# Vasilispapg/CVML-GoalNet

Measured on AMD Instinct MI355X. Metric: training clips/sec at batch 64, 16-frame 224² clips; logit MAE vs CPU ref, higher is better.
Workload: dtype f32; 1 GPU; AVM train step (forward + broadcast-MSE + backward + fused Adam), 64 clips x 16 frames = 1024 frames of 3x224x224 + 30x30 MFCC per GPU; dropout live (device masks), BatchNorm train mode; frames_per_gpu=1024, h=224, w=224, parallelism=dp1, ddp_semantics=local BN + local MSE per rank, gradient mean (standard DDP), params=1286754369

## Files before the change

cvml_goalnet_amd/csrc/gemm_f32.hip:

```cpp
#include <stdlib.h>

#include "gemm_common.h"
#include "skinny.h"

using namespace goalnet;

namespace {

constexpr int BM = 128, BN = 128, BK = 32;
constexpr int LDR = 128;
constexpr int OP_FLOATS = BM * BK;

__device__ __forceinline__ int kc_off(int row, int chunk) { return row * BK + ((chunk ^ ((row >> 1) & 7)) << 2); }

__device__ __forceinline__ float4 f4zero() { return make_float4(0.f, 0.f, 0.f, 0.f); }
__device__ __forceinline__ float4 f4fma(float4 v, float4 s, float4 t) {
    return make_float4(fmaf(v.x, s.x, t.x), fmaf(v.y, s.y, t.y), fmaf(v.z, s.z, t.z), fmaf(v.w, s.w, t.w));
}

typedef unsigned int u32x4 __attribute__((ext_vector_type(4)));
constexpr unsigned OOB = 0xFFFFFF00u;

__device__ __forceinline__ float4 f4sel(bool v, float4 a) { return v ? a : f4zero(); }

__device__ __forceinline__ __amdgpu_buffer_rsrc_t make_rsrc(const void* base, uint32_t bytes) {
    return __builtin_amdgcn_make_buffer_rsrc(const_cast<void*>(base), 0, (int)bytes, 0x00020000);
}
__device__ __forceinline__ float4 bload(__amdgpu_buffer_rsrc_t r, unsigned voff, unsigned soff) {
    const u32x4 v = __builtin_amdgcn_raw_buffer_load_b128(r, (int)voff, (int)soff, 0);
    return make_float4(__uint_as_float(v.x), __uint_as_float(v.y), __uint_as_float(v.z), __uint_as_float(v.w));
}
__device__ __forceinline__ uint32_t clamp_u32(int64_t v) {
    return v <= 0 ? 0u : (v > 0xFFFFFF00ll ? 0xFFFFFF00u : (uint32_t)v);
}

template <bool AFFINE>
struct KCLoader {
    struct P {
        const float* x; int64_t ld; int rows;
        const float* scale; const float* shift; int bnC;
        int convC;
    };
    static constexpr bool KC = true;
    static constexpr bool ONE_STAGE = false;
    static constexpr int ONE_STAGE_BLOCKS = 3;
    __amdgpu_buffer_rsrc_t rx, rsc, rsh;
    unsigned voff[4], vaff;
    int bnC, convC;
    float4 sc, sh;
    __device__ KCLoader(const P& p, int row0, int tid) {
        const int nrows = p.rows - row0 < BM ? p.rows - row0 : BM;
        rx = make_rsrc(p.x + (int64_t)row0 * p.ld, clamp_u32((int64_t)nrows * p.ld * 4));
#pragma unroll
        for (int i = 0; i < 4; ++i) {
            const int rl = (tid >> 3) + 32 * i;
            voff[i] = rl < nrows ? (unsigned)(((int64_t)rl * p.ld + (tid & 7) * 4) * 4) : OOB;
        }
        bnC = p.bnC; convC = p.convC;
        if (AFFINE) {
            rsc = make_rsrc(p.scale, (uint32_t)p.bnC * 4);
            rsh = make_rsrc(p.shift, (uint32_t)p.bnC * 4);
            vaff = (unsigned)((tid & 7) * 16);
        }
    }
    __device__ __forceinline__ void issue(int kt, float4 (&r)[4]) {
        unsigned k4 = (unsigned)kt * (BK * 4);
        if (convC > 0) {
            const int chunk = kt / 9, tap = kt - 9 * chunk;
            k4 = (unsigned)(tap * convC + chunk * BK) * 4;
        }
        if (AFFINE) {
            const unsigned ch4 = (unsigned)((kt * BK) % bnC) * 4;
            sc = bload(rsc, vaff, ch4);
            sh = bload(rsh, vaff, ch4);
        }
#pragma unroll
        for (int i = 0; i < 4; ++i) r[i] = bload(rx, voff[i], k4);
    }
    __device__ __forceinline__ void finish(float4 (&r)[4]) const {
        if (AFFINE) {
#pragma unroll
            for (int i = 0; i < 4; ++i) r[i] = f4fma(r[i], sc, sh);
        }
    }
};

template <bool AFFINE>
struct MCLoader {
    struct P {
        const float* x; int64_t ld; int cols; int kred;
        const float* scale; const float* shift; int bnC;
    };
    static constexpr bool KC = false;
    static constexpr bool ONE_STAGE = true;
#ifndef GN_MC_BLOCKS
#define GN_MC_BLOCKS 4
#endif
    static constexpr int ONE_STAGE_BLOCKS = GN_MC_BLOCKS;
    const float* x;
    int64_t ld;
    int kred, k0;
    unsigned voff[4];
    bool partial;
    float4 sc, sh;
    __device__ MCLoader(const P& p, int col0, int tid) {
        const int col = col0 + (tid & 31) * 4;
        const bool colok = col < p.cols;
        x = p.x; ld = p.ld; kred = p.kred; k0 = tid >> 5;
#pragma unroll
        for (int i = 0; i < 4; ++i) voff[i] = colok ? (unsigned)(((int64_t)(k0 + 8 * i) * p.ld + col) * 4) : OOB;
        partial = false;
        if (AFFINE) {
            const int ch = (colok ? col : 0) % p.bnC;
            sc = *reinterpret_cast<const float4*>(p.scale + ch);
            sh = *reinterpret_cast<const float4*>(p.shift + ch);
            if (!colok) sh = f4zero();
        }
    }
    __device__ __forceinline__ void issue(int kt, float4 (&r)[4]) {
        const int kbase = kt * BK;
        const int nk = kred - kbase < BK ? kred - kbase : BK;
        partial = nk < BK;
        const __amdgpu_buffer_rsrc_t rx = make_rsrc(x + (int64_t)kbase * ld, clamp_u32((int64_t)nk * ld * 4));
#pragma unroll
        for (int i = 0; i < 4; ++i) r[i] = bload(rx, voff[i], 0);
    }
    __device__ __forceinline__ void finish(float4 (&r)[4]) const {
        if (AFFINE) {
            if (partial) {
#pragma unroll
                for (int i = 0; i < 4; ++i) r[i] = f4sel(k0 + 8 * i < (kred & (BK - 1)), f4fma(r[i], sc, sh));
            } else {
#pragma unroll
                for (int i = 0; i < 4; ++i) r[i] = f4fma(r[i], sc, sh);
            }
        }
    }
};

template <bool AFFINE>
struct ConvALoader {
    struct P {
        const float* x; int H, W, C; int64_t M;
        const float* scale; const float* shift;
    };
    static constexpr bool KC = true;
    static constexpr bool ONE_STAGE = true;
    static constexpr int ONE_STAGE_BLOCKS = AFFINE ? 3 : 4;
    __amdgpu_buffer_rsrc_t rx, rsc, rsh;
    unsigned mask[4];
    unsigned voff, vaff, vmask;
    int W, C;
    float4 sc, sh;
    __device__ ConvALoader(const P& p, int row0, int tid) {
        W = p.W; C = p.C;
        const int c4 = (tid & 7) * 4, rr = tid >> 3;
        rx = make_rsrc(p.x + ((int64_t)row0 - (p.W + 1)) * p.C, (uint32_t)((BM + 2 * (p.W + 1)) * p.C * 4));
        voff = (unsigned)((rr * p.C + c4) * 4);
        if (AFFINE) {
            rsc = make_rsrc(p.scale, (uint32_t)p.C * 4);
            rsh = make_rsrc(p.shift, (uint32_t)p.C * 4);
            vaff = (unsigned)(c4 * 4);
        }
#pragma unroll
        for (int i = 0; i < 4; ++i) {
            const int64_t m = (int64_t)row0 + rr + 32 * i;
            unsigned mk = 0;
            if (m < p.M) {
                const int w = (int)((unsigned)m % (unsigned)p.W);
                const int h = (int)(((unsigned)m / (unsigned)p.W) % (unsigned)p.H);
#pragma unroll
                for (int kh = 0; kh < 3; ++kh)
#pragma unroll
                    for (int kw = 0; kw < 3; ++kw) {
                        const bool v = (unsigned)(h + kh - 1) < (unsigned)p.H && (unsigned)(w + kw - 1) < (unsigned)p.W;
                        mk |= (v ? 1u : 0u) << (kh * 3 + kw);
                    }
            }
            mask[i] = mk;
        }
    }
    __device__ __forceinline__ void issue(int kt, float4 (&r)[4]) {
        const int chunk = kt / 9;
        const int tap = kt - 9 * chunk;
        const int ci = chunk * BK;
        const int kh = tap / 3, kw = tap - 3 * kh;
        const unsigned s0 = (unsigned)(((kh * W + kw) * C + ci) * 4);
        const unsigned rowstep = (unsigned)(32 * C * 4);
        if (AFFINE) {
            sc = bload(rsc, vaff, (unsigned)ci * 4);
            sh = bload(rsh, vaff, (unsigned)ci * 4);
        }
        vmask = 0;
#pragma unroll
        for (int i = 0; i < 4; ++i) {
            const bool v = (mask[i] >> tap) & 1u;
            vmask |= (v ? 1u : 0u) << i;
            r[i] = bload(rx, v ? voff : OOB, s0 + (unsigned)i * rowstep);
        }
    }
    __device__ __forceinline__ void finish(float4 (&r)[4]) const {
        if (AFFINE) {
#pragma unroll
            for (int i = 0; i < 4; ++i) r[i] = f4sel((vmask >> i) & 1u, f4fma(r[i], sc, sh));
        }
    }
};

template <bool AFFINE, bool DSEL = false>
struct ConvWgradBLoader {
    struct P {
        const float* x; int H, W, C; int M;
        const float* scale; const float* shift;
        const uint32_t* codes4;
    };
    static constexpr bool KC = false;
    const float* x;
    __amdgpu_buffer_rsrc_t rcodes;
    int W, C, M, k0, tapshift, nextkt;
    unsigned voff[4], bad4, nextcode, badnow;
    float4 sc, sh;
    __device__ ConvWgradBLoader(const P& p, int col0, int tid) {
        const int col = col0 + (tid & 31) * 4;
        const bool colok = col < 9 * p.C;
        const int cc = colok ? col : 0;
        const int tap = cc / p.C, ci = cc - tap * p.C;
        const int kh = tap / 3, kw = tap - 3 * kh;
        x = p.x; W = p.W; C = p.C; M = p.M; k0 = tid >> 5;
        rcodes = make_rsrc(p.codes4, (uint32_t)((p.M + 31) / 32 * 32));
        bad4 = ((kh == 0 ? 1u : 0u) | (kh == 2 ? 2u : 0u) | (kw == 0 ? 4u : 0u) | (kw == 2 ? 8u : 0u)) * 0x01010101u;
        tapshift = kh * p.W + kw;
        nextkt = -1; nextcode = 0;
#pragma unroll
        for (int i = 0; i < 4; ++i) voff[i] = colok ? (unsigned)(((k0 + 8 * i + tapshift) * p.C + ci) * 4) : OOB;
        if (AFFINE) {
            sc = *reinterpret_cast<const float4*>(p.scale + ci);
            sh = *reinterpret_cast<const float4*>(p.shift + ci);
        }
    }
    __device__ __forceinline__ unsigned load_code(int kt) const {
        return (unsigned)__builtin_amdgcn_raw_buffer_load_b32(rcodes, k0 * 4, kt * 32, 0);
    }
    __device__ __forceinline__ void issue(int kt, float4 (&r)[4]) {
        const int mbase = kt * BK;
        const unsigned badc = (nextkt == kt ? nextcode : load_code(kt)) & bad4;
        badnow = badc;
        const unsigned bad = DSEL ? 0u : badc;
        const int64_t lead = (int64_t)mbase - (W + 1);
        const int64_t last = (int64_t)mbase + BK + (W + 1) < M ? (int64_t)mbase + BK + (W + 1) : M;
        const __amdgpu_buffer_rsrc_t rx = make_rsrc(x + lead * C, clamp_u32((last - lead) * C * 4));
        if (lead < 0) {
#pragma unroll
            for (int i = 0; i < 4; ++i)
                r[i] = bload(rx, (mbase + k0 + 8 * i + tapshift < W + 1 || ((bad >> (8 * i)) & 0xFFu)) ? OOB : voff[i], 0);
        } else {
#pragma unroll
            for (int i = 0; i < 4; ++i) r[i] = bload(rx, ((bad >> (8 * i)) & 0xFFu) ? OOB : voff[i], 0);
        }
        nextcode = load_code(kt + 1);
        nextkt = kt + 1;
    }
    __device__ __forceinline__ void finish(float4 (&r)[4]) const {
        if (DSEL) {
#pragma unroll
            for (int i = 0; i < 4; ++i) r[i] = f4sel(((badnow >> (8 * i)) & 0xFFu) == 0, AFFINE ? f4fma(r[i], sc, sh) : r[i]);
        } else if (AFFINE) {
#pragma unroll
            for (int i = 0; i < 4; ++i) r[i] = f4fma(r[i], sc, sh);
        }
    }
};

__global__ __launch_bounds__(256) void border_codes_kernel(uint32_t* __restrict__ codes4, int M, int Mpad, int H, int W) {
    for (int j = blockIdx.x * blockDim.x + threadIdx.x; j < Mpad / 4; j += gridDim.x * blockDim.x) {
        const int kt = j >> 3, k0 = j & 7;
        uint32_t word = 0;
#pragma unroll
        for (int i = 0; i < 4; ++i) {
            const int m = kt * 32 + k0 + 8 * i;
            const int w = m % W, h = (m / W) % H;
            const uint32_t c = m < M ? (uint32_t)((h == 0 ? 1 : 0) | (h == H - 1 ? 2 : 0) | (w == 0 ? 4 : 0) | (w == W - 1 ? 8 : 0)) : 0xFu;
            word |= c << (8 * i);
        }
        codes4[j] = word;
    }
}

__global__ __launch_bounds__(256) void wgrad_border_sums_kernel(const float* __restrict__ dy, double* __restrict__ parts,
                                                               int H, int W, int Cout) {
    const int n = blockIdx.x;
    const float* f = dy + (int64_t)n * H * W * Cout;
    double* out = parts + (int64_t)n * 8 * Cout;
    for (int c = threadIdx.x; c < Cout; c += blockDim.x) {
        double r0 = 0, r1 = 0, c0 = 0, c1 = 0;
        for (int w = 0; w < W; ++w) { r0 += (double)f[(int64_t)w * Cout + c]; r1 += (double)f[((int64_t)(H - 1) * W + w) * Cout + c]; }
        for (int h = 0; h < H; ++h) { c0 += (double)f[(int64_t)h * W * Cout + c]; c1 += (double)f[((int64_t)h * W + W - 1) * Cout + c]; }
        out[0 * Cout + c] = r0; out[1 * Cout + c] = r1; out[2 * Cout + c] = c0; out[3 * Cout + c] = c1;
        out[4 * Cout + c] = (double)f[c];
        out[5 * Cout + c] = (double)f[(int64_t)(W - 1) * Cout + c];
        out[6 * Cout + c] = (double)f[(int64_t)(H - 1) * W * Cout + c];
        out[7 * Cout + c] = (double)f[((int64_t)(H - 1) * W + W - 1) * Cout + c];
    }
}

__device__ __forceinline__ float border_u_of(const double* v, int tap) {
    const int kh = tap / 3, kw = tap - 3 * kh;
    double r = (kh == 0 ? v[0] : 0.0) + (kh == 2 ? v[1] : 0.0) + (kw == 0 ? v[2] : 0.0) + (kw == 2 ? v[3] : 0.0);
    if (kh == 0 && kw == 0) r -= v[4];
    if (kh == 0 && kw == 2) r -= v[5];
    if (kh == 2 && kw == 0) r -= v[6];
    if (kh == 2 && kw == 2) r -= v[7];
    return (float)r;
}

__global__ __launch_bounds__(256) void wgrad_border_u_kernel(const double* __restrict__ parts, int N, int Cout, float* __restrict__ u) {
    __shared__ double s[32][8];
    const int cl = threadIdx.x & 31, j = threadIdx.x >> 5;
    const int c = blockIdx.x * 32 + cl;
    double a0 = 0, a1 = 0, a2 = 0, a3 = 0;
    if (c < Cout) {
        const double* q = parts + (int64_t)j * Cout + c;
        int n = 0;
        for (; n + 3 < N; n += 4) {
            a0 += q[(int64_t)n * 8 * Cout]; a1 += q[(int64_t)(n + 1) * 8 * Cout];
            a2 += q[(int64_t)(n + 2) * 8 * Cout]; a3 += q[(int64_t)(n + 3) * 8 * Cout];
        }
        for (; n < N; ++n) a0 += q[(int64_t)n * 8 * Cout];
    }
    s[cl][j] = (a0 + a1) + (a2 + a3);
    __syncthreads();
    for (int t = threadIdx.x; t < 32 * 9; t += 256) {
        const int cc = t / 9, tap = t - 9 * cc;
        if (blockIdx.x * 32 + cc < Cout) u[(int64_t)(blockIdx.x * 32 + cc) * 9 + tap] = border_u_of(s[cc], tap);
    }
}

template <bool KC>
__device__ __forceinline__ void store_tile(float* l, const float4 (&r)[4], int tid) {
    if (KC) {
        const int c4 = (tid & 7) * 4, row = tid >> 3;
#pragma unroll
        for (int i = 0; i < 4; ++i) *reinterpret_cast<float4*>(&l[kc_off(row + 32 * i, c4 >> 2)]) = r[i];
    } else {
        const int r4 = (tid & 31) * 4, k = tid >> 5;
#pragma unroll
        for (int i = 0; i < 4; ++i) *reinterpret_cast<float4*>(&l[(k + 8 * i) * LDR + r4]) = r[i];
    }
}

template <bool KC>
__device__ __forceinline__ void read_group(const float* l, int strip, int s, int r, int h, float (&f)[2][4]) {
    if (KC) {
#pragma unroll
        for (int q = 0; q < 2; ++q) {
            const float4 t = *reinterpret_cast<const float4*>(&l[kc_off(strip + q * 32 + r, 2 * s + h)]);
            f[q][0] = t.x; f[q][1] = t.y; f[q][2] = t.z; f[q][3] = t.w;
        }
    } else {
#pragma unroll
        for (int j = 0; j < 4; ++j) {
            const float2 t = *reinterpret_cast<const float2*>(&l[(8 * s + 4 * h + j) * LDR + strip + 2 * r]);
            f[0][j] = t.x; f[1][j] = t.y;
        }
    }
}

template <bool AKC, bool BKC>
__device__ __forceinline__ void compute_tile(const float* la, const float* lb, f32x16 (&acc)[2][2],
                                             int wm, int wn, int r, int h) {
#pragma unroll
    for (int s = 0; s < 4; ++s) {
        float a[2][4], b[2][4];
        read_group<AKC>(la, wm * 64, s, r, h, a);
        read_group<BKC>(lb, wn * 64, s, r, h, b);
#pragma unroll
        for (int j = 0; j < 4; ++j) {
#pragma unroll
            for (int fm = 0; fm < 2; ++fm)
#pragma unroll
                for (int fn = 0; fn < 2; ++fn)
                    acc[fm][fn] = __builtin_amdgcn_mfma_f32_32x32x2f32(a[fm][j], b[fn][j], acc[fm][fn], 0, 0, 0);
        }
    }
}

__device__ __forceinline__ void compute_tile_n64(const float* la, const float* lb, f32x16 (&acc)[2], int wave, int r, int h) {
#pragma unroll
    for (int s = 0; s < 4; ++s) {
        const float4 ta = *reinterpret_cast<const float4*>(&la[kc_off(wave * 32 + r, 2 * s + h)]);
        const float4 tb0 = *reinterpret_cast<const float4*>(&lb[kc_off(r, 2 * s + h)]);
        const float4 tb1 = *reinterpret_cast<const float4*>(&lb[kc_off(32 + r, 2 * s + h)]);
        const float a[4] = {ta.x, ta.y, ta.z, ta.w}, b0[4] = {tb0.x, tb0.y, tb0.z, tb0.w}, b1[4] = {tb1.x, tb1.y, tb1.z, tb1.w};
#pragma unroll
        for (int j = 0; j < 4; ++j) {
            acc[0] = __builtin_amdgcn_mfma_f32_32x32x2f32(a[j], b0[j], acc[0], 0, 0, 0);
            acc[1] = __builtin_amdgcn_mfma_f32_32x32x2f32(a[j], b1[j], acc[1], 0, 0, 0);
        }
    }
}

__device__ __forceinline__ void store_acc_n64(const EpiP& ep, const f32x16 (&acc)[2], int tm, int tn, int split, int wave, int r, int h) {
    float* outp = ep.slab_stride > 0 ? (ep.slabs ? ep.slabs : ep.out) + (int64_t)split * ep.slab_stride : ep.out;
    const int mode = ep.slab_stride > 0 ? EPI_RAW : ep.mode;
    const int64_t ld = (ep.slab_stride > 0 && ep.slabs) ? (int64_t)ep.cols : ep.ld;
#pragma unroll
    for (int fn = 0; fn < 2; ++fn) {
        const int col = tn * 64 + fn * 32 + r;
        const bool colok = col < ep.cols;
        const int64_t row0 = (int64_t)tm * BM + wave * 32 + 4 * h;
        const float bv = (mode == EPI_BIAS_RELU && ep.bias) ? ep.bias[colok ? col : 0] : 0.f;
        const float lo = (mode == EPI_BIAS_RELU && ep.relu) ? 0.f : -INFINITY;
#pragma unroll
        for (int e = 0; e < 16; ++e) {
            const int64_t row = row0 + (e & 3) + 8 * (e >> 2);
            if (!(colok && row < ep.rows)) continue;
            const float v = acc[fn][e];
            if (mode == EPI_RAW) outp[row * ld + col] = v;
            else if (mode == EPI_BIAS_RELU) outp[row * ld + col] = fmaxf(v + bv, lo);
            else outp[row * ld + col] = epi_apply(ep, v, row, col);
        }
    }
}

template <class AL, class BL, bool N64 = false, int STAGES = 2>
__global__ __launch_bounds__(256, STAGES == 1 ? (N64 ? 4 : AL::ONE_STAGE_BLOCKS) : 2) void gemm_f32_kernel(typename AL::P ap, typename BL::P bp, EpiP ep,
                                                          int tiles_m, int tiles_n, int m_fast,
                                                          int ktiles, int ktiles_per_split, int xcd_splits) {
    __shared__ __attribute__((aligned(16))) float lds[STAGES][2][OP_FLOATS];
    const int tid = threadIdx.x;
    int tm, tn, split;
    if (xcd_splits > 0) {
        const int tiles = tiles_m * tiles_n;
        const int xcd = blockIdx.x & 7, j = blockIdx.x >> 3;
        int t;
        if (tiles > 64 && tiles <= 128) {
            const int gs = (xcd_splits + 7) / 8, rest = tiles - 64, nA = gs * 64;
            int q;
            if (j < nA) { q = j >> 6; t = j & 63; }
            else { const int i = j - nA; q = i / rest; t = 64 + (i - q * rest); }
            split = q * 8 + xcd;
        } else {
            split = (j / tiles) * 8 + xcd;
            t = j - (j / tiles) * tiles;
        }
        if (split >= xcd_splits) return;
        if (m_fast) { tm = t % tiles_m; tn = t / tiles_m; } else { tn = t % tiles_n; tm = t / tiles_n; }
    } else {
        tile_of_block(tiles_m, tiles_n, m_fast, tm, tn);
        split = blockIdx.y;
    }
    const int kt0 = split * ktiles_per_split;
    const int kt1 = min(ktiles, kt0 + ktiles_per_split);

    static_assert(!N64 || (AL::KC && BL::KC), "the 128 x 64 tile reads K-contiguous LDS images");
    AL al(ap, tm * BM, tid);
    BL bl(bp, tn * (N64 ? 64 : BN), tid);

    const int lane = tid & 63, wave = tid >> 6;
    const int wm = wave >> 1, wn = wave & 1;
    const int r = lane & 31, h = lane >> 5;

    f32x16 acc[2][2];
#pragma unroll
    for (int i = 0; i < 2; ++i)
#pragma unroll
        for (int j = 0; j < 2; ++j)
#pragma unroll
            for (int e = 0; e < 16; ++e) acc[i][j][e] = 0.f;

    float4 ra[4], rb[4];
    if (kt0 < kt1) {
        al.issue(kt0, ra);
        bl.issue(kt0, rb);
        al.finish(ra);
        bl.finish(rb);
        store_tile<AL::KC>(lds[0][0], ra, tid);
        store_tile<BL::KC>(lds[0][1], rb, tid);
    }
    __syncthreads();
    for (int kt = kt0; kt < kt1; ++kt) {
        const int cur = STAGES == 1 ? 0 : (kt - kt0) & 1;
        const bool more = kt + 1 < kt1;
        if (more) {
            al.issue(kt + 1, ra);
            bl.issue(kt + 1, rb);
        }
        if constexpr (N64) compute_tile_n64(lds[cur][0], lds[cur][1], acc[0], wave, r, h);
        else compute_tile<AL::KC, BL::KC>(lds[cur][0], lds[cur][1], acc, wm, wn, r, h);
        if constexpr (STAGES == 1) __syncthreads();
        if (more) {
            al.finish(ra);
            bl.finish(rb);
            store_tile<AL::KC>(lds[STAGES == 1 ? 0 : cur ^ 1][0], ra, tid);
            store_tile<BL::KC>(lds[STAGES == 1 ? 0 : cur ^ 1][1], rb, tid);
        }
        __syncthreads();
    }
    if constexpr (N64) store_acc_n64(ep, acc[0], tm, tn, split, wave, r, h);
    else store_acc<!AL::KC, !BL::KC>(ep, acc, tm, tn, split, wm, wn, r, h);
    if (ep.tile_ctr) {
        const int nsp = (ktiles + ktiles_per_split - 1) / ktiles_per_split;
        fused_splitk_reduce<N64 ? 64 : BN>(ep, tm, tn, tm * tiles_n + tn, nsp, tid);
    }
}

__global__ __launch_bounds__(256) void splitk_reduce_kernel(const float* slabs, int nsplit, int64_t slab_stride, EpiP ep) {
    const int c4n = ep.cols >> 2;
    const int64_t total = (int64_t)ep.rows * c4n;
    for (int64_t i = (int64_t)blockIdx.x * blockDim.x + threadIdx.x; i < total; i += (int64_t)gridDim.x * blockDim.x) {
        const int64_t row = i / c4n;
        const int col = (int)(i - row * c4n) * 4;
        const float* s = slabs + row * ep.cols + col;
        float4 a = *reinterpret_cast<const float4*>(s);
        for (int k = 1; k < nsplit; ++k) {
            const float4 b = *reinterpret_cast<const float4*>(s + (int64_t)k * slab_stride);
            a.x += b.x; a.y += b.y; a.z += b.z; a.w += b.w;
        }
        if (ep.oscale) { const int k = *ep.oscale; a.x = ldexpf(a.x, k); a.y = ldexpf(a.y, k); a.z = ldexpf(a.z, k); a.w = ldexpf(a.w, k); }
        if (ep.corr_u) {
            const int tap = col / ep.corr_C, ci = col - tap * ep.corr_C;
            const float u = ep.corr_u[row * 9 + tap];
            const float4 shv = *reinterpret_cast<const float4*>(ep.corr_sh + ci);
            a.x = fmaf(-shv.x, u, a.x); a.y = fmaf(-shv.y, u, a.y); a.z = fmaf(-shv.z, u, a.z); a.w = fmaf(-shv.w, u, a.w);
        }
        float* o = ep.out + row * ep.ld + col;
        o[0] = epi_apply(ep, a.x, row, col);
        o[1] = epi_apply(ep, a.y, row, col + 1);
        o[2] = epi_apply(ep, a.z, row, col + 2);
        o[3] = epi_apply(ep, a.w, row, col + 3);
    }
}

__global__ __launch_bounds__(256) void splitk_reduce_wide_kernel(const float* slabs, int nsplit, int64_t slab_stride, EpiP ep) {
    const int c4n = ep.cols >> 2;
    const int64_t total = (int64_t)ep.rows * c4n;
    const int g = threadIdx.x & 15;
    const int64_t step = (int64_t)gridDim.x * 16;
    const int64_t rounds = (total + step - 1) / step;
    int64_t i = (int64_t)blockIdx.x * 16 + (threadIdx.x >> 4);
    for (int64_t r = 0; r < rounds; ++r, i += step) {
        const bool ok = i < total;
        const int64_t ic = ok ? i : 0;
        const int64_t row = ic / c4n;
        const int col = (int)(ic - row * c4n) * 4;
        const float* s = slabs + row * ep.cols + col;
        float4 a = make_float4(0.f, 0.f, 0.f, 0.f);
        for (int k = g; k < nsplit; k += 16) {
            const float4 b = *reinterpret_cast<const float4*>(s + (int64_t)k * slab_stride);
            a.x += b.x; a.y += b.y; a.z += b.z; a.w += b.w;
        }
        a.x = row16_sum(a.x); a.y = row16_sum(a.y); a.z = row16_sum(a.z); a.w = row16_sum(a.w);
        if (ep.oscale) { const int k = *ep.oscale; a.x = ldexpf(a.x, k); a.y = ldexpf(a.y, k); a.z = ldexpf(a.z, k); a.w = ldexpf(a.w, k); }
        if (ep.corr_u) {
            const int tap = col / ep.corr_C, ci = col - tap * ep.corr_C;
            const float u = ep.corr_u[row * 9 + tap];
            const float4 shv = *reinterpret_cast<const float4*>(ep.corr_sh + ci);
            a.x = fmaf(-shv.x, u, a.x); a.y = fmaf(-shv.y, u, a.y); a.z = fmaf(-shv.z, u, a.z); a.w = fmaf(-shv.w, u, a.w);
        }
        if (ok && g == 0) {
            float* o = ep.out + row * ep.ld + col;
            o[0] = epi_apply(ep, a.x, row, col);
            o[1] = epi_apply(ep, a.y, row, col + 1);
            o[2] = epi_apply(ep, a.z, row, col + 2);
            o[3] = epi_apply(ep, a.w, row, col + 3);
        }
    }
}

template <class AL, class BL, bool N64 = false>
int launch_gemm(const char* name, const typename AL::P& ap, const typename BL::P& bp, const EpiP& ep,
                int64_t M, int64_t N, int ktiles, int nsplit, int m_fast, hipStream_t st) {
    const int64_t tiles_m = (M + BM - 1) / BM, tiles_n = (N + (N64 ? 64 : BN) - 1) / (N64 ? 64 : BN);
    GN_REQUIRE(tiles_m * tiles_n < (1ll << 31), GOALNET_E_SHAPE, "%s: too many tiles", name);
    GN_REQUIRE(nsplit >= 1 && nsplit <= 65535, GOALNET_E_SHAPE, "%s: bad split count %d", name, nsplit);
    const int kps = (ktiles + nsplit - 1) / nsplit;
    GN_REQUIRE(!ep.tile_ctr || (ktiles + kps - 1) / kps == nsplit, GOALNET_E_SHAPE, "%s: fused split-K needs every split non-empty", name);
    const bool xcd_local = nsplit >= 8 && tiles_m * tiles_n <= 256 && tiles_m * tiles_n * ((nsplit + 7) / 8 * 8) < (1ll << 31);
    dim3 grid((unsigned)(tiles_m * tiles_n), (unsigned)nsplit, 1);
    if (xcd_local) grid = dim3((unsigned)(tiles_m * tiles_n * ((nsplit + 7) / 8 * 8)), 1, 1);
    static const int force_stages = getenv("GOALNET_F32_STAGES") ? atoi(getenv("GOALNET_F32_STAGES")) : 0;
    const bool one_stage = force_stages == 1 || (force_stages != 2 && AL::ONE_STAGE);
    if (one_stage) {
        hipLaunchKernelGGL((gemm_f32_kernel<AL, BL, N64, 1>), grid, dim3(256), 0, st, ap, bp, ep, (int)tiles_m, (int)tiles_n,
                           m_fast, ktiles, kps, xcd_local ? nsplit : 0);
        GN_LAUNCH_CHECK(name);
        return 0;
    }
    hipLaunchKernelGGL((gemm_f32_kernel<AL, BL, N64>), grid, dim3(256), 0, st, ap, bp, ep, (int)tiles_m, (int)tiles_n,
                       m_fast, ktiles, kps, xcd_local ? nsplit : 0);
    GN_LAUNCH_CHECK(name);
    return 0;
}

}

namespace goalnet {
int launch_splitk_reduce(const char* name, const float* slabs, int nsplit, int64_t slab_stride, const EpiP& ep, hipStream_t st) {
    const int64_t total = (int64_t)ep.rows * (ep.cols >> 2);
    int64_t blocks = (total + 255) / 256;
    if (blocks > 4096) blocks = 4096;
    if (blocks < 1) blocks = 1;
    if (total < 65536 && nsplit >= 32) {
        int64_t wb = (total + 15) / 16;
        if (wb > 4096) wb = 4096;
        hipLaunchKernelGGL(splitk_reduce_wide_kernel, dim3((unsigned)wb), dim3(256), 0, st, slabs, nsplit, slab_stride, ep);
        GN_LAUNCH_CHECK(name);
        return 0;
    }
    hipLaunchKernelGGL(splitk_reduce_kernel, dim3((unsigned)blocks), dim3(256), 0, st, slabs, nsplit, slab_stride, ep);
    GN_LAUNCH_CHECK(name);
    return 0;
}

int pick_splits(int64_t tiles, int ktiles) {
    if (ktiles < 8 || (ktiles < 64 && tiles >= 128)) return 1;
    int64_t s = ((ktiles < 64 ? 256 : 1024) + tiles - 1) / tiles;
    const int64_t smax = ktiles < 64 ? ktiles / 4 : (ktiles / 8 > 1 ? ktiles / 8 : 1);
    if (s > smax) s = smax;
    if (s < 1) s = 1;
    const int kps = (int)((ktiles + s - 1) / s);
    return (ktiles + kps - 1) / kps;
}

}

extern "C" {

static int conv_splits_f32(int64_t M, int Cin, int Cout) {
    return conv_fwd_splits(((M + BM - 1) / BM) * ((Cout + BN - 1) / BN), 9 * Cin / BK);
}

size_t goalnet_conv3x3_fwd_ws_bytes(int N, int H, int W, int Cin, int Cout) {
    if (N <= 0 || H <= 0 || W <= 0 || Cin <= 0 || Cout <= 0) return 0;
    const int64_t M = (int64_t)N * H * W;
    const int s = conv_splits_f32(M, Cin, Cout);
    return s > 1 ? (size_t)s * (size_t)M * (size_t)Cout * sizeof(float) : 0;
}

int goalnet_conv3x3_fwd(const float* x, const float* scale, const float* shift, const float* w,
                        const float* bias, int relu, float* y, int N, int H, int W, int Cin, int Cout,
                        void* ws, size_t ws_bytes, int* tile_ctr, int n_ctr, void* stream) {
    GN_REQUIRE(x && w && y, GOALNET_E_NULL, "conv3x3_fwd: null pointer");
    GN_REQUIRE((scale == nullptr) == (shift == nullptr), GOALNET_E_NULL, "conv3x3_fwd: scale/shift must both be set or both NULL");
    GN_REQUIRE(N > 0 && H > 0 && W > 0 && Cin > 0 && Cout > 0, GOALNET_E_SHAPE, "conv3x3_fwd: non-positive dim");
    GN_REQUIRE(Cin % BK == 0, GOALNET_E_SHAPE, "conv3x3_fwd: Cin=%d must be a multiple of %d", Cin, BK);
    GN_REQUIRE(Cout % 4 == 0, GOALNET_E_SHAPE, "conv3x3_fwd: Cout=%d must be a multiple of 4", Cout);
    GN_REQUIRE(aligned16(x) && aligned16(w) && aligned16(y) && aligned16(scale) && aligned16(shift),
               GOALNET_E_ALIGN, "conv3x3_fwd: pointers must be 16-byte aligned");
    const int64_t M = (int64_t)N * H * W;
    GN_REQUIRE(M < (1ll << 31) - 256, GOALNET_E_SHAPE, "conv3x3_fwd: N*H*W too large");
    hipStream_t st = (hipStream_t)stream;
    KCLoader<false>::P bp{w, (int64_t)9 * Cin, Cout, nullptr, nullptr, 1, Cin};
    const EpiP efinal{EPI_BIAS_RELU, y, Cout, (int)M, Cout, bias, relu, nullptr, 0, nullptr, 0, 0};
    EpiP ep = efinal;
    const int ktiles = 9 * Cin / BK;
    int nsplit = ws ? conv_splits_f32(M, Cin, Cout) : 1;
    if (nsplit > 1) {
        GN_REQUIRE(aligned16(ws) && ws_bytes >= goalnet_conv3x3_fwd_ws_bytes(N, H, W, Cin, Cout), GOALNET_E_WORKSPACE,
                   "conv3x3_fwd: workspace too small or misaligned");
        ep = EpiP{EPI_RAW, (float*)ws, Cout, (int)M, Cout, nullptr, 0, nullptr, 0, nullptr, 0, M * Cout};
    }
    const bool narrow = Cout <= 64 && !getenv("GOALNET_F32_N64_OFF");
    const bool fused = nsplit > 1 && tile_ctr && (int64_t)n_ctr >= ((M + BM - 1) / BM) * ((Cout + (narrow ? 64 : BN) - 1) / (narrow ? 64 : BN));
    if (fused) {
        ep = efinal;
        ep.slabs = (float*)ws; ep.slab_stride = M * Cout; ep.tile_ctr = tile_ctr;
    }
    int rc;
    if (scale) {
        ConvALoader<true>::P ap{x, H, W, Cin, M, scale, shift};
        rc = narrow ? launch_gemm<ConvALoader<true>, KCLoader<false>, true>("conv3x3_fwd", ap, bp, ep, M, Cout, ktiles, nsplit, 0, st)
                    : launch_gemm<ConvALoader<true>, KCLoader<false>>("conv3x3_fwd", ap, bp, ep, M, Cout, ktiles, nsplit, 0, st);
    } else {
        ConvALoader<false>::P ap{x, H, W, Cin, M, nullptr, nullptr};
        rc = narrow ? launch_gemm<ConvALoader<false>, KCLoader<false>, true>("conv3x3_fwd", ap, bp, ep, M, Cout, ktiles, nsplit, 0, st)
                    : launch_gemm<ConvALoader<false>, KCLoader<false>>("conv3x3_fwd", ap, bp, ep, M, Cout, ktiles, nsplit, 0, st);
    }
    if (rc || nsplit == 1 || fused) return rc;
    return launch_splitk_reduce("conv3x3_fwd.reduce", (const float*)ws, nsplit, M * Cout, efinal, st);
}

}
namespace {
template <class AL, class BL, bool N64, int STAGES> const char* gemm_f32_kernel_name_() { return __PRETTY_FUNCTION__; }
template <class AL, class BL, bool N64> const char* gemm_f32_kernel_name() {
    const int force = getenv("GOALNET_F32_STAGES") ? atoi(getenv("GOALNET_F32_STAGES")) : 0;
    const bool one = force == 1 || (force != 2 && AL::ONE_STAGE);
    return one ? gemm_f32_kernel_name_<AL, BL, N64, 1>() : gemm_f32_kernel_name_<AL, BL, N64, 2>();
}
}
extern "C" {

const char* goalnet_conv3x3_fwd_kernel_name(int N, int H, int W, int Cin, int Cout, int affine) {
    (void)N; (void)H; (void)W; (void)Cin;
    const bool narrow = Cout <= 64 && !getenv("GOALNET_F32_N64_OFF");
    if (affine) return narrow ? gemm_f32_kernel_name<ConvALoader<true>, KCLoader<false>, true>() : gemm_f32_kernel_name<ConvALoader<true>, KCLoader<false>, false>();
    return narrow ? gemm_f32_kernel_name<ConvALoader<false>, KCLoader<false>, true>() : gemm_f32_kernel_name<ConvALoader<false>, KCLoader<false>, false>();
}

static int wgrad_splits(int64_t M, int Cin, int Cout) {
    const int64_t tiles = (int64_t)((Cout + BM - 1) / BM) * ((9 * Cin + BN - 1) / BN);
    const int ktiles = (int)((M + BK - 1) / BK);
    static const int wtarget = getenv("GOALNET_WGRAD_SPLIT_TARGET") ? atoi(getenv("GOALNET_WGRAD_SPLIT_TARGET")) : 2048;
    int64_t s = (wtarget + tiles - 1) / tiles;
    const int64_t smax = ktiles / 4 > 1 ? ktiles / 4 : 1;
    if (s > smax) s = smax;
    if (s > 512) s = 512;
    if (s >= 8) {
        int64_t best = (s + 7) / 8 * 8 <= smax ? (s + 7) / 8 * 8 : s / 8 * 8;
        double best_eff = 0.0;
        for (int64_t c = best; c <= 2 * s + 8 && c <= smax && c <= 1024; c += 8) {
            const int64_t blocks = tiles * c, rounds = (blocks + 511) / 512;
            const double eff = (double)blocks / (double)(rounds * 512);
            if (eff > best_eff + 1e-9) { best_eff = eff; best = c; }
        }
        s = best;
    }
    const int kps = (int)((ktiles + s - 1) / s);
    return (ktiles + kps - 1) / kps;
}

static size_t wgrad_codes_bytes(int64_t M) { return (size_t)((M + 31) / 32 * 32 + 255) / 256 * 256; }
static size_t wgrad_border_bytes(int N, int Cout) {
    return ((size_t)N * 8 * Cout * sizeof(double) + 255) / 256 * 256 + ((size_t)Cout * 9 * sizeof(float) + 255) / 256 * 256;
}

size_t goalnet_conv3x3_wgrad_ws_bytes(int N, int H, int W, int Cin, int Cout) {
    const int64_t M = (int64_t)N * H * W;
    return wgrad_codes_bytes(M) + wgrad_border_bytes(N, Cout) + (size_t)wgrad_splits(M, Cin, Cout) * (size_t)Cout * 9 * Cin * sizeof(float);
}

int goalnet_conv3x3_wgrad_codes(uint32_t* codes, int N, int H, int W, void* stream) {
    GN_REQUIRE(codes && N > 0 && H > 0 && W > 0, GOALNET_E_NULL, "conv3x3_wgrad_codes: bad arguments");
    const int64_t M = (int64_t)N * H * W;
    GN_REQUIRE(M < (1ll << 31) - 256, GOALNET_E_SHAPE, "conv3x3_wgrad_codes: N*H*W too large");
    const int Mpad = (int)((M + 31) / 32 * 32);
    int blocks = (Mpad / 4 + 255) / 256;
    if (blocks > 4096) blocks = 4096;
    hipLaunchKernelGGL(border_codes_kernel, dim3(blocks), dim3(256), 0, (hipStream_t)stream, codes, (int)M, Mpad, H, W);
    GN_LAUNCH_CHECK("conv3x3_wgrad_codes");
    return 0;
}

size_t goalnet_conv3x3_wgrad_codes_bytes(int N, int H, int W) { return wgrad_codes_bytes((int64_t)N * H * W); }

int goalnet_conv3x3_wgrad(const float* x, const float* scale, const float* shift, const float* dy, float* dw,
                          void* ws, size_t ws_bytes, const uint32_t* codes_in, int* tile_ctr, int n_ctr,
                          int N, int H, int W, int Cin, int Cout, void* stream) {
    GN_REQUIRE(x && dy && dw && ws, GOALNET_E_NULL, "conv3x3_wgrad: null pointer");
    GN_REQUIRE((scale == nullptr) == (shift == nullptr), GOALNET_E_NULL, "conv3x3_wgrad: scale/shift must both be set or both NULL");
    GN_REQUIRE(N > 0 && H > 0 && W > 0, GOALNET_E_SHAPE, "conv3x3_wgrad: non-positive dim");
    GN_REQUIRE(Cin % 4 == 0 && Cout % 4 == 0 && Cin > 0 && Cout > 0, GOALNET_E_SHAPE, "conv3x3_wgrad: channels must be multiples of 4");
    GN_REQUIRE(aligned16(x) && aligned16(dy) && aligned16(dw) && aligned16(ws) && aligned16(scale) && aligned16(shift),
               GOALNET_E_ALIGN, "conv3x3_wgrad: pointers must be 16-byte aligned");
    const int64_t M = (int64_t)N * H * W;
    GN_REQUIRE(M < (1ll << 31) - 256, GOALNET_E_SHAPE, "conv3x3_wgrad: N*H*W too large");
    GN_REQUIRE(ws_bytes >= goalnet_conv3x3_wgrad_ws_bytes(N, H, W, Cin, Cout), GOALNET_E_WORKSPACE, "conv3x3_wgrad: workspace too small");
    hipStream_t st = (hipStream_t)stream;
    const int nsplit = wgrad_splits(M, Cin, Cout);
    const int ktiles = (int)((M + BK - 1) / BK);
    const int64_t slab = (int64_t)Cout * 9 * Cin;
    uint32_t* codes = (uint32_t*)ws;
    double* bparts = (double*)((char*)ws + wgrad_codes_bytes(M));
    float* bu = (float*)((char*)bparts + ((size_t)N * 8 * Cout * sizeof(double) + 255) / 256 * 256);
    float* slabs = (float*)((char*)ws + wgrad_codes_bytes(M) + wgrad_border_bytes(N, Cout));
    const char* force = getenv("GOALNET_WGRAD_PATH");
    const bool dsel = force && force[0] == 's' ? true : force && force[0] == 'c' ? false : (int64_t)N * (H > W ? H : W) <= 4096;
    if (codes_in) {
        codes = const_cast<uint32_t*>(codes_in);
    } else {
        const int Mpad = (int)((M + 31) / 32 * 32);
        int blocks = (Mpad / 4 + 255) / 256;
        if (blocks > 4096) blocks = 4096;
        hipLaunchKernelGGL(border_codes_kernel, dim3(blocks), dim3(256), 0, st, codes, (int)M, Mpad, H, W);
        GN_LAUNCH_CHECK("conv3x3_wgrad.codes");
    }
    if (scale && !dsel) {
        hipLaunchKernelGGL(wgrad_border_sums_kernel, dim3(N), dim3(256), 0, st, dy, bparts, H, W, Cout);
        GN_LAUNCH_CHECK("conv3x3_wgrad.border_sums");
        hipLaunchKernelGGL(wgrad_border_u_kernel, dim3((Cout + 31) / 32), dim3(256), 0, st, bparts, N, Cout, bu);
        GN_LAUNCH_CHECK("conv3x3_wgrad.border_u");
    }
    MCLoader<false>::P ap{dy, Cout, Cout, (int)M, nullptr, nullptr, 1};
    EpiP ep{EPI_RAW, slabs, (int64_t)9 * Cin, Cout, 9 * Cin, nullptr, 0, nullptr, 0, nullptr, 0, slab};
    const bool fused = nsplit > 1 && tile_ctr && (dsel || !scale) &&
                       (int64_t)n_ctr >= (int64_t)((Cout + BM - 1) / BM) * ((9 * Cin + BN - 1) / BN);
    if (fused) {
        ep = EpiP{EPI_RAW, dw, (int64_t)9 * Cin, Cout, 9 * Cin, nullptr, 0, nullptr, 0, nullptr, 0, slab};
        ep.slabs = slabs; ep.tile_ctr = tile_ctr;
    }
    int rc;
    if (scale && dsel) {
        ConvWgradBLoader<true, true>::P bp{x, H, W, Cin, (int)M, scale, shift, codes};
        rc = launch_gemm<MCLoader<false>, ConvWgradBLoader<true, true>>("conv3x3_wgrad", ap, bp, ep, Cout, 9 * Cin, ktiles, nsplit, 1, st);
    } else if (scale) {
        ConvWgradBLoader<true>::P bp{x, H, W, Cin, (int)M, scale, shift, codes};
        rc = launch_gemm<MCLoader<false>, ConvWgradBLoader<true>>("conv3x3_wgrad", ap, bp, ep, Cout, 9 * Cin, ktiles, nsplit, 1, st);
    } else {
        ConvWgradBLoader<false>::P bp{x, H, W, Cin, (int)M, nullptr, nullptr, codes};
        rc = launch_gemm<MCLoader<false>, ConvWgradBLoader<false>>("conv3x3_wgrad", ap, bp, ep, Cout, 9 * Cin, ktiles, nsplit, 1, st);
    }
    if (rc || fused) return rc;
    EpiP er{EPI_RAW, dw, (int64_t)9 * Cin, Cout, 9 * Cin, nullptr, 0, nullptr, 0, nullptr, 0, 0};
    if (scale && !dsel) { er.corr_u = bu; er.corr_sh = shift; er.corr_C = Cin; }
    return launch_splitk_reduce("conv3x3_wgrad.reduce", slabs, nsplit, slab, er, st);
}

static int linear_splits(int M, int64_t K, int J) {
    const int64_t tiles = (int64_t)((M + BM - 1) / BM) * ((J + BN - 1) / BN);
    return pick_splits(tiles, (int)(K / BK));
}

size_t goalnet_linear_fwd_ws_bytes(int M, int64_t K, int J) {
    if (M <= 0 || K <= 0 || J <= 0) return 0;
    if (M <= SKINNY_MAX_M) return skinny_fwd_ws_bytes(M, K, J);
    const int s = linear_splits(M, K, J);
    return s > 1 ? (size_t)s * (size_t)M * (size_t)J * sizeof(float) : 0;
}

int goalnet_linear_fwd(const float* x, int64_t ldx, const float* scale, const float* shift, int bnC,
                       const float* w, const float* bias, int relu, const float* dropmask, int64_t ldmask,
                       float* y, int64_t ldy, float* mult_out, int64_t ldmult,
                       int M, int64_t K, int J, void* ws, size_t ws_bytes, void* stream) {
    GN_REQUIRE(x && w && y, GOALNET_E_NULL, "linear_fwd: null pointer");
    GN_REQUIRE((scale == nullptr) == (shift == nullptr), GOALNET_E_NULL, "linear_fwd: scale/shift must both be set or both NULL");
    GN_REQUIRE(M > 0 && J > 0 && K > 0 && K < (1ll << 31) - 64, GOALNET_E_SHAPE, "linear_fwd: bad dims");
    GN_REQUIRE(K % BK == 0, GOALNET_E_SHAPE, "linear_fwd: K=%lld must be a multiple of %d", (long long)K, BK);
    GN_REQUIRE(J % 4 == 0, GOALNET_E_SHAPE, "linear_fwd: J=%d must be a multiple of 4", J);
    GN_REQUIRE(!scale || (bnC > 0 && bnC % 4 == 0), GOALNET_E_SHAPE, "linear_fwd: bnC must be a positive multiple of 4");
    GN_REQUIRE(aligned16(x) && aligned16(w) && aligned16(y) && aligned16(scale) && aligned16(shift) && ldx % 4 == 0 && ldy % 4 == 0,
               GOALNET_E_ALIGN, "linear_fwd: pointers / leading dims must be 16-byte aligned");
    hipStream_t st = (hipStream_t)stream;
    EpiP efinal{(dropmask || mult_out) ? EPI_FULL : EPI_BIAS_RELU, y, ldy, M, J, bias, relu, dropmask, ldmask, mult_out, ldmult, 0};
    if (M <= SKINNY_MAX_M) {
        const size_t need = skinny_fwd_ws_bytes(M, K, J);
        GN_REQUIRE(need == 0 || (ws && aligned16(ws) && ws_bytes >= need), GOALNET_E_WORKSPACE, "linear_fwd: workspace too small");
        return skinny_linear_fwd(x, ldx, scale, shift, bnC, w, efinal, M, K, J, ws, st);
    }
    const int nsplit = linear_splits(M, K, J);
    const int ktiles = (int)(K / BK);
    KCLoader<false>::P bp{w, K, J, nullptr, nullptr, 1, 0};
    EpiP ep = efinal;
    if (nsplit > 1) {
        GN_REQUIRE(ws && aligned16(ws), GOALNET_E_WORKSPACE, "linear_fwd: split-K needs a 16-byte aligned workspace");
        GN_REQUIRE(ws_bytes >= goalnet_linear_fwd_ws_bytes(M, K, J), GOALNET_E_WORKSPACE, "linear_fwd: workspace too small");
        ep = EpiP{EPI_RAW, (float*)ws, J, M, J, nullptr, 0, nullptr, 0, nullptr, 0, (int64_t)M * J};
    }
    int rc;
// ... 54 lines not shown
```

Measured before the change: 154.0 clips/s.

## Add LDS strip loader reusing halo rows across 3x3 conv taps

Adds a strip-based A loader for the implicit-GEMM 3x3 conv forward. It stages a 288-row input strip (tile plus halo) into LDS once per channel chunk, and all nine taps then read from that strip with a per-tap row shift and a zero pad row. The current loader re-fetches global memory for every tap. The aim is to cut redundant global loads by roughly nine times for narrow feature maps without split-K. In exchange, LDS use per block rises, occupancy is fixed at one stage with fewer blocks, and each tap needs two barriers.

```diff
diff --git a/cvml_goalnet_amd/csrc/gemm_f32.hip b/cvml_goalnet_amd/csrc/gemm_f32.hip
--- a/cvml_goalnet_amd/csrc/gemm_f32.hip
+++ b/cvml_goalnet_amd/csrc/gemm_f32.hip
@@ -42,6 +42,7 @@
         int convC;
     };
     static constexpr bool KC = true;
+    static constexpr bool STRIP = false;
     static constexpr bool ONE_STAGE = false;
     static constexpr int ONE_STAGE_BLOCKS = 3;
     __amdgpu_buffer_rsrc_t rx, rsc, rsh;
@@ -92,6 +93,7 @@
         const float* scale; const float* shift; int bnC;
     };
     static constexpr bool KC = false;
+    static constexpr bool STRIP = false;
     static constexpr bool ONE_STAGE = true;
 #ifndef GN_MC_BLOCKS
 #define GN_MC_BLOCKS 4
@@ -138,6 +140,22 @@
     }
 };
 
+__device__ __forceinline__ unsigned conv_tap_mask(int64_t m, int64_t M, int H, int W) {
+    unsigned mk = 0;
+    if (m < M) {
+        const int w = (int)((unsigned)m % (unsigned)W);
+        const int h = (int)(((unsigned)m / (unsigned)W) % (unsigned)H);
+#pragma unroll
+        for (int kh = 0; kh < 3; ++kh)
+#pragma unroll
+            for (int kw = 0; kw < 3; ++kw) {
+                const bool v = (unsigned)(h + kh - 1) < (unsigned)H && (unsigned)(w + kw - 1) < (unsigned)W;
+                mk |= (v ? 1u : 0u) << (kh * 3 + kw);
+            }
+    }
+    return mk;
+}
+
 template <bool AFFINE>
 struct ConvALoader {
     struct P {
@@ -145,6 +163,7 @@
         const float* scale; const float* shift;
     };
     static constexpr bool KC = true;
+    static constexpr bool STRIP = false;
     static constexpr bool ONE_STAGE = true;
     static constexpr int ONE_STAGE_BLOCKS = AFFINE ? 3 : 4;
     __amdgpu_buffer_rsrc_t rx, rsc, rsh;
@@ -164,20 +183,7 @@
         }
 #pragma unroll
         for (int i = 0; i < 4; ++i) {
-            const int64_t m = (int64_t)row0 + rr + 32 * i;
-            unsigned mk = 0;
-            if (m < p.M) {
-                const int w = (int)((unsigned)m % (unsigned)p.W);
-                const int h = (int)(((unsigned)m / (unsigned)p.W) % (unsigned)p.H);
-#pragma unroll
-                for (int kh = 0; kh < 3; ++kh)
-#pragma unroll
-                    for (int kw = 0; kw < 3; ++kw) {
-                        const bool v = (unsigned)(h + kh - 1) < (unsigned)p.H && (unsigned)(w + kw - 1) < (unsigned)p.W;
-                        mk |= (v ? 1u : 0u) << (kh * 3 + kw);
-                    }
-            }
-            mask[i] = mk;
+            mask[i] = conv_tap_mask((int64_t)row0 + rr + 32 * i, p.M, p.H, p.W);
         }
     }
     __device__ __forceinline__ void issue(int kt, float4 (&r)[4]) {
@@ -203,6 +209,80 @@
         if (AFFINE) {
 #pragma unroll
             for (int i = 0; i < 4; ++i) r[i] = f4sel((vmask >> i) & 1u, f4fma(r[i], sc, sh));
+        }
+    }
+};
+
+constexpr int STRIP_LOADS = 9;
+constexpr int STRIP_ROWS = 32 * STRIP_LOADS;
+constexpr int STRIP_FLOATS = (STRIP_ROWS + 1) * BK;
+constexpr int CONV_STRIP_MAX_W = (STRIP_ROWS - BM) / 2 - 1;
+
+template <bool AFFINE>
+struct ConvAStripLoader {
+    using P = typename ConvALoader<AFFINE>::P;
+    static constexpr bool KC = true;
+    static constexpr bool STRIP = true;
+    static constexpr bool ONE_STAGE = true;
+    static constexpr int ONE_STAGE_BLOCKS = 3;
+    __amdgpu_buffer_rsrc_t rx, rsc, rsh;
+    unsigned mask[2];
+    unsigned lrow[2];
+    unsigned voff, vaff, bad;
+    int W, C, h;
+    float4 sc, sh;
+    __device__ ConvAStripLoader(const P& p, int row0, int tid) {
+        W = p.W; C = p.C;
+        const int c4 = (tid & 7) * 4, rr = tid >> 3;
+        const int64_t lead = (int64_t)row0 - (p.W + 1);
+        const int nrows = BM + 2 * (p.W + 1);
+        rx = make_rsrc(p.x + lead * p.C, (uint32_t)(nrows * p.C * 4));
+        voff = (unsigned)((rr * p.C + c4) * 4);
+        bad = 0;
+#pragma unroll
+        for (int i = 0; i < STRIP_LOADS; ++i) {
+            const int64_t pix = lead + rr + 32 * i;
+            bad |= (pix < 0 || pix >= p.M || rr + 32 * i >= nrows ? 1u : 0u) << i;
+        }
+        if (AFFINE) {
+            rsc = make_rsrc(p.scale, (uint32_t)p.C * 4);
+            rsh = make_rsrc(p.shift, (uint32_t)p.C * 4);
+            vaff = (unsigned)(c4 * 4);
+        }
+        const int wm = tid >> 7, r = tid & 31;
+        h = (tid >> 5) & 1;
+#pragma unroll
+        for (int q = 0; q < 2; ++q) {
+            lrow[q] = (unsigned)(wm * 64 + q * 32 + r);
+            mask[q] = conv_tap_mask((int64_t)row0 + lrow[q], p.M, p.H, p.W);
+        }
+    }
+    __device__ __forceinline__ void begin(int chunk) {
+        if (AFFINE) {
+            sc = bload(rsc, vaff, (unsigned)(chunk * BK) * 4);
+            sh = bload(rsh, vaff, (unsigned)(chunk * BK) * 4);
+        }
+    }
+    __device__ __forceinline__ float4 load(int chunk, int i) const {
+        unsigned b = bad;
+        asm volatile("" : "+v"(b));
+        return bload(rx, (b >> i) & 1u ? OOB : voff, (unsigned)((i * 32 * C + chunk * BK) * 4));
+    }
+    __device__ __forceinline__ void store(float* l, const float4 (&rs)[STRIP_LOADS], int tid) const {
+        const int c = tid & 7, row = tid >> 3;
+#pragma unroll
+        for (int i = 0; i < STRIP_LOADS; ++i)
+            *reinterpret_cast<float4*>(&l[kc_off(row + 32 * i, c)]) = AFFINE ? f4fma(rs[i], sc, sh) : rs[i];
+    }
+    __device__ __forceinline__ void frag_base(int tap, unsigned (&ab)[2]) const {
+        const int kh = tap / 3, kw = tap - 3 * kh;
+        const unsigned shift = (unsigned)(kh * W + kw);
+#pragma unroll
+        for (int q = 0; q < 2; ++q) {
+            unsigned mk = mask[q];
+            asm volatile("" : "+v"(mk));
+            const unsigned row = (mk >> tap) & 1u ? lrow[q] + shift : (unsigned)STRIP_ROWS;
+            ab[q] = (row << 7) | (((unsigned)h ^ ((row >> 1) & 7u)) << 4);
         }
     }
 };
@@ -384,6 +464,70 @@
     }
 }
 
+template <bool BKC>
+__device__ __forceinline__ void compute_tile_strip(const float* ls, const float* lb, f32x16 (&acc)[2][2],
+                                                   const unsigned (&ab)[2], int wn, int r, int h) {
+    static_assert(BKC, "K-contiguous B image");
+    const unsigned bb = (unsigned)kc_off(wn * 64 + r, h) * 4;
+#pragma unroll
+    for (int s = 0; s < 4; ++s) {
+        float a[2][4], b[2][4];
+#pragma unroll
+        for (int q = 0; q < 2; ++q) {
+            const float4 t = *reinterpret_cast<const float4*>(reinterpret_cast<const char*>(ls) + (ab[q] ^ (unsigned)(s << 5)));
+            a[q][0] = t.x; a[q][1] = t.y; a[q][2] = t.z; a[q][3] = t.w;
+            const float4 u = *reinterpret_cast<const float4*>(reinterpret_cast<const char*>(lb) + ((bb ^ (unsigned)(s << 5)) + q * 32 * BK * 4));
+            b[q][0] = u.x; b[q][1] = u.y; b[q][2] = u.z; b[q][3] = u.w;
+        }
+#pragma unroll
+        for (int j = 0; j < 4; ++j) {
+#pragma unroll
+            for (int fm = 0; fm < 2; ++fm)
+#pragma unroll
+                for (int fn = 0; fn < 2; ++fn)
+                    acc[fm][fn] = __builtin_amdgcn_mfma_f32_32x32x2f32(a[fm][j], b[fn][j], acc[fm][fn], 0, 0, 0);
+        }
+    }
+}
+
+template <class AL, class BL>
+__device__ __forceinline__ void conv_strip_loop(AL& al, BL& bl, float* ls, float* lb, f32x16 (&acc)[2][2], int ktiles,
+                                                int tid, int wn, int r, int h) {
+    float4 rs[STRIP_LOADS], rb[4];
+    const int nchunks = ktiles / 9;
+    if (tid < 8) *reinterpret_cast<float4*>(&ls[STRIP_ROWS * BK + tid * 4]) = f4zero();
+    al.begin(0);
+#pragma unroll
+    for (int i = 0; i < STRIP_LOADS; ++i) rs[i] = al.load(0, i);
+    bl.issue(0, rb);
+    al.store(ls, rs, tid);
+    bl.finish(rb);
+    store_tile<BL::KC>(lb, rb, tid);
+    __syncthreads();
+    for (int chunk = 0; chunk < nchunks; ++chunk) {
+        const bool next = chunk + 1 < nchunks;
+#pragma unroll
+        for (int tap = 0; tap < 9; ++tap) {
+            const bool more = tap < 8 || next;
+            if (more) bl.issue(chunk * 9 + tap + 1, rb);
+            if (next) rs[tap] = al.load(chunk + 1, tap);
+            unsigned ab[2];
+            al.frag_base(tap, ab);
+            compute_tile_strip<BL::KC>(ls, lb, acc, ab, wn, r, h);
+            __syncthreads();
+            if (more) {
+                bl.finish(rb);
+                store_tile<BL::KC>(lb, rb, tid);
+            }
+            if (tap == 8 && next) {
+                al.begin(chunk + 1);
+                al.store(ls, rs, tid);
+            }
+            __syncthreads();
+        }
+    }
+}
+
 __device__ __forceinline__ void compute_tile_n64(const float* la, const float* lb, f32x16 (&acc)[2], int wave, int r, int h) {
 #pragma unroll
     for (int s = 0; s < 4; ++s) {
@@ -426,7 +570,6 @@
 __global__ __launch_bounds__(256, STAGES == 1 ? (N64 ? 4 : AL::ONE_STAGE_BLOCKS) : 2) void gemm_f32_kernel(typename AL::P ap, typename BL::P bp, EpiP ep,
                                                           int tiles_m, int tiles_n, int m_fast,
                                                           int ktiles, int ktiles_per_split, int xcd_splits) {
-    __shared__ __attribute__((aligned(16))) float lds[STAGES][2][OP_FLOATS];
     const int tid = threadIdx.x;
     int tm, tn, split;
     if (xcd_splits > 0) {
@@ -468,33 +611,41 @@
 #pragma unroll
             for (int e = 0; e < 16; ++e) acc[i][j][e] = 0.f;
 
-    float4 ra[4], rb[4];
-    if (kt0 < kt1) {
-        al.issue(kt0, ra);
-        bl.issue(kt0, rb);
-        al.finish(ra);
-        bl.finish(rb);
-        store_tile<AL::KC>(lds[0][0], ra, tid);
-        store_tile<BL::KC>(lds[0][1], rb, tid);
-    }
-    __syncthreads();
-    for (int kt = kt0; kt < kt1; ++kt) {
-        const int cur = STAGES == 1 ? 0 : (kt - kt0) & 1;
-        const bool more = kt + 1 < kt1;
-        if (more) {
-            al.issue(kt + 1, ra);
-            bl.issue(kt + 1, rb);
-        }
-        if constexpr (N64) compute_tile_n64(lds[cur][0], lds[cur][1], acc[0], wave, r, h);
-        else compute_tile<AL::KC, BL::KC>(lds[cur][0], lds[cur][1], acc, wm, wn, r, h);
-        if constexpr (STAGES == 1) __syncthreads();
-        if (more) {
+    if constexpr (AL::STRIP) {
+        static_assert(!N64 && STAGES == 1 && BL::KC, "the strip form: 128 x 128 tile, one B stage");
+        __shared__ __attribute__((aligned(16))) float lstrip[STRIP_FLOATS];
+        __shared__ __attribute__((aligned(16))) float lbs[OP_FLOATS];
+        conv_strip_loop(al, bl, lstrip, lbs, acc, kt1 - kt0, tid, wn, r, h);
+    } else {
+        __shared__ __attribute__((aligned(16))) float lds[STAGES][2][OP_FLOATS];
+        float4 ra[4], rb[4];
+        if (kt0 < kt1) {
+            al.issue(kt0, ra);
+            bl.issue(kt0, rb);
             al.finish(ra);
             bl.finish(rb);
-            store_tile<AL::KC>(lds[STAGES == 1 ? 0 : cur ^ 1][0], ra, tid);
-            store_tile<BL::KC>(lds[STAGES == 1 ? 0 : cur ^ 1][1], rb, tid);
+            store_tile<AL::KC>(lds[0][0], ra, tid);
+            store_tile<BL::KC>(lds[0][1], rb, tid);
         }
         __syncthreads();
+        for (int kt = kt0; kt < kt1; ++kt) {
+            const int cur = STAGES == 1 ? 0 : (kt - kt0) & 1;
+            const bool more = kt + 1 < kt1;
+            if (more) {
+                al.issue(kt + 1, ra);
+                bl.issue(kt + 1, rb);
+            }
+            if constexpr (N64) compute_tile_n64(lds[cur][0], lds[cur][1], acc[0], wave, r, h);
+            else compute_tile<AL::KC, BL::KC>(lds[cur][0], lds[cur][1], acc, wm, wn, r, h);
+            if constexpr (STAGES == 1) __syncthreads();
+            if (more) {
+                al.finish(ra);
+                bl.finish(rb);
+                store_tile<AL::KC>(lds[STAGES == 1 ? 0 : cur ^ 1][0], ra, tid);
+                store_tile<BL::KC>(lds[STAGES == 1 ? 0 : cur ^ 1][1], rb, tid);
+            }
+            __syncthreads();
+        }
     }
     if constexpr (N64) store_acc_n64(ep, acc[0], tm, tn, split, wave, r, h);
     else store_acc<!AL::KC, !BL::KC>(ep, acc, tm, tn, split, wm, wn, r, h);
@@ -579,16 +730,18 @@
     dim3 grid((unsigned)(tiles_m * tiles_n), (unsigned)nsplit, 1);
     if (xcd_local) grid = dim3((unsigned)(tiles_m * tiles_n * ((nsplit + 7) / 8 * 8)), 1, 1);
     static const int force_stages = getenv("GOALNET_F32_STAGES") ? atoi(getenv("GOALNET_F32_STAGES")) : 0;
-    const bool one_stage = force_stages == 1 || (force_stages != 2 && AL::ONE_STAGE);
+    const bool one_stage = AL::STRIP || force_stages == 1 || (force_stages != 2 && AL::ONE_STAGE);
     if (one_stage) {
         hipLaunchKernelGGL((gemm_f32_kernel<AL, BL, N64, 1>), grid, dim3(256), 0, st, ap, bp, ep, (int)tiles_m, (int)tiles_n,
                            m_fast, ktiles, kps, xcd_local ? nsplit : 0);
         GN_LAUNCH_CHECK(name);
         return 0;
     }
-    hipLaunchKernelGGL((gemm_f32_kernel<AL, BL, N64>), grid, dim3(256), 0, st, ap, bp, ep, (int)tiles_m, (int)tiles_n,
-                       m_fast, ktiles, kps, xcd_local ? nsplit : 0);
-    GN_LAUNCH_CHECK(name);
+    if constexpr (!AL::STRIP) {
+        hipLaunchKernelGGL((gemm_f32_kernel<AL, BL, N64>), grid, dim3(256), 0, st, ap, bp, ep, (int)tiles_m, (int)tiles_n,
+                           m_fast, ktiles, kps, xcd_local ? nsplit : 0);
+        GN_LAUNCH_CHECK(name);
+    }
     return 0;
 }
 
@@ -628,6 +781,14 @@
 
 static int conv_splits_f32(int64_t M, int Cin, int Cout) {
     return conv_fwd_splits(((M + BM - 1) / BM) * ((Cout + BN - 1) / BN), 9 * Cin / BK);
+}
+
+constexpr bool CONV_STRIP_FWD = true;
+constexpr bool CONV_STRIP_DGRAD = true;
+static bool conv_strip_f32(int W, int nsplit, bool narrow, bool affine) {
+    const char* e = getenv("GOALNET_F32_CONV_STRIP");
+    if (e && e[0] == '0') return false;
+    return nsplit == 1 && !narrow && W <= CONV_STRIP_MAX_W && (affine ? CONV_STRIP_FWD : CONV_STRIP_DGRAD);
 }
 
 size_t goalnet_conv3x3_fwd_ws_bytes(int N, int H, int W, int Cin, int Cout) {
@@ -666,8 +827,15 @@
         ep = efinal;
         ep.slabs = (float*)ws; ep.slab_stride = M * Cout; ep.tile_ctr = tile_ctr;
     }
+    const bool strip = conv_strip_f32(W, nsplit, narrow, scale != nullptr);
     int rc;
-    if (scale) {
+    if (strip && scale) {
+        ConvAStripLoader<true>::P ap{x, H, W, Cin, M, scale, shift};
+        rc = launch_gemm<ConvAStripLoader<true>, KCLoader<false>>("conv3x3_fwd", ap, bp, ep, M, Cout, ktiles, 1, 0, st);
+    } else if (strip) {
+        ConvAStripLoader<false>::P ap{x, H, W, Cin, M, nullptr, nullptr};
+        rc = launch_gemm<ConvAStripLoader<false>, KCLoader<false>>("conv3x3_fwd", ap, bp, ep, M, Cout, ktiles, 1, 0, st);
+    } else if (scale) {
         ConvALoader<true>::P ap{x, H, W, Cin, M, scale, shift};
         rc = narrow ? launch_gemm<ConvALoader<true>, KCLoader<false>, true>("conv3x3_fwd", ap, bp, ep, M, Cout, ktiles, nsplit, 0, st)
                     : launch_gemm<ConvALoader<true>, KCLoader<false>>("conv3x3_fwd", ap, bp, ep, M, Cout, ktiles, nsplit, 0, st);
@@ -685,15 +853,18 @@
 template <class AL, class BL, bool N64, int STAGES> const char* gemm_f32_kernel_name_() { return __PRETTY_FUNCTION__; }
 template <class AL, class BL, bool N64> const char* gemm_f32_kernel_name() {
     const int force = getenv("GOALNET_F32_STAGES") ? atoi(getenv("GOALNET_F32_STAGES")) : 0;
-    const bool one = force == 1 || (force != 2 && AL::ONE_STAGE);
+    const bool one = AL::STRIP || force == 1 || (force != 2 && AL::ONE_STAGE);
     return one ? gemm_f32_kernel_name_<AL, BL, N64, 1>() : gemm_f32_kernel_name_<AL, BL, N64, 2>();
 }
 }
 extern "C" {
 
 const char* goalnet_conv3x3_fwd_kernel_name(int N, int H, int W, int Cin, int Cout, int affine) {
-    (void)N; (void)H; (void)W; (void)Cin;
     const bool narrow = Cout <= 64 && !getenv("GOALNET_F32_N64_OFF");
+    const int nsplit = (N > 0 && H > 0 && W > 0 && Cin > 0 && Cout > 0) ? conv_splits_f32((int64_t)N * H * W, Cin, Cout) : 1;
+    if (conv_strip_f32(W, nsplit, narrow, affine != 0))
+        return affine ? gemm_f32_kernel_name<ConvAStripLoader<true>, KCLoader<false>, false>()
+                      : gemm_f32_kernel_name<ConvAStripLoader<false>, KCLoader<false>, false>();
     if (affine) return narrow ? gemm_f32_kernel_name<ConvALoader<true>, KCLoader<false>, true>() : gemm_f32_kernel_name<ConvALoader<true>, KCLoader<false>, false>();
     return narrow ? gemm_f32_kernel_name<ConvALoader<false>, KCLoader<false>, true>() : gemm_f32_kernel_name<ConvALoader<false>, KCLoader<false>, false>();
 }
```

Result: faster. 157.1 clips/s, median of 6 (+2.0%).
